# ascentai/diy-gym

Measured on NVIDIA B200. Metric: aggregate env-steps/sec, higher is better.
Workload: dtype f32

## Files before the change

### diy_gym_b200/csrc/dg_env.cuh

```cuda
#pragma once
#include "dg_math.cuh"
#include "dg_scene.h"

namespace dg {

struct Env {
  const DevScene* sc;
  float* ws;
  float* wg;
  float* st;
  float* pr;
  const float* act;
  float* obs;
  float* rew;
  uint8_t* term;
  const int* link_i;
  const float* link_f;
  const float* link_x;
  uint32_t seed;
  int env_id;
  bool active;
  int grp0, grp1;
  unsigned long long opmask[2];
  unsigned long long* dbg;
// ... 58 lines not shown
    float* K = KIN(s);
    q_to_mat(K, ST(S_BQUAT) + 4 * f); v_cpy(K + 9, ST(S_BPOS) + 3 * f);
  }
  if (ln == 0) for (int i = 0; i < WH_COUNT; i++) WSI(C)[sc.W_HDR + i] = 0;
}

DG_FN void joint_xform(const Env& C, int gl, float q, float* E, float* r) {
  const int* li = shc(C.link_i) + DG_LINK_I_W * gl; const float* lf = shc(C.link_f) + DG_LINK_F_W * gl; const float* R0 = shc(C.link_x) + 16 * gl;
  float Rrel[9], tmp[3];
  if (li[2] == 1) { float Ra[9]; axis_angle_mat(Ra, lf + 10, q, C.sc->precise != 0); m_mul(Rrel, R0, Ra); m_vec(tmp, Rrel, lf + 7); }
  else if (li[2] == 2) { m_cpy(Rrel, R0); float dd[3] = {lf[7] + lf[10] * q, lf[8] + lf[11] * q, lf[9] + lf[12] * q}; m_vec(tmp, R0, dd); }
  else { m_cpy(Rrel, R0); m_vec(tmp, R0, lf + 7); }
  v_add(r, lf + 4, tmp);
  E[0] = Rrel[0]; E[1] = Rrel[3]; E[2] = Rrel[6]; E[3] = Rrel[1]; E[4] = Rrel[4]; E[5] = Rrel[7]; E[6] = Rrel[2]; E[7] = Rrel[5]; E[8] = Rrel[8];
}
DG_HD int parent_slot(const int* li, int l0, int s0) { return li[1] < 0 ? s0 : s0 + 1 + (li[1] - l0); }

struct F4 { float x, y, z, w; };
DG_HD F4 ld4(const float* p) {
#if defined(__CUDA_ARCH__)
  float4 v = *reinterpret_cast<const float4*>(p); F4 o = {v.x, v.y, v.z, v.w}; return o;
#else
  F4 o = {p[0], p[1], p[2], p[3]}; return o;
#endif
}
DG_HD void st4(float* p, float x, float y, float z, float w) {
#if defined(__CUDA_ARCH__)
  *reinterpret_cast<float4*>(p) = make_float4(x, y, z, w);
#else
  p[0] = x; p[1] = y; p[2] = z; p[3] = w;
#endif
}
template <int N> DG_HD void ldn(const float* p, float* o) {
#pragma unroll
  for (int c = 0; c < N / 4; c++) { F4 v = ld4(p + 4 * c); o[4 * c] = v.x; o[4 * c + 1] = v.y; o[4 * c + 2] = v.z; o[4 * c + 3] = v.w; }
}
template <int N> DG_HD void stn(float* p, const float* v) {
#pragma unroll
  for (int c = 0; c < N / 4; c++) st4(p + 4 * c, v[4 * c], v[4 * c + 1], v[4 * c + 2], v[4 * c + 3]);
}

template <bool BIAS>
DG_FN void fk_vel_body(const Env& C, int b) {
  const DevScene& sc = SC;
  const int* bi = gc(sc.body_i) + DG_BODY_I_W * b; const int* bp = gc(sc.body_plan) + BP_W * b;
  const int kind = bi[0], l0 = bi[1], nlb = bi[2], s0 = bp[BP_SLOT];
  const float* bs = BST(bp[BP_DI]);
  const float *mass = PR(P_MASS), *inertia = PR(P_INERTIA);
  const float kl = PR(P_LINDAMP)[b], ka = PR(P_ANGDAMP)[b];
  float Kp[12], Vp[6];
  q_to_mat(Kp, bs + 3); v_cpy(Kp + 9, bs);
  mT_vec(Vp, Kp, bs + 10); mT_vec(Vp + 3, Kp, bs + 7);
  int prev = s0;
  for (int k = -1; k < nlb; k++) {
    const int s = s0 + 1 + k, f = k < 0 ? b : sc.nb + l0 + k;
    float K[12], V[6], cacc[8] = {0, 0, 0, 0, 0, 0, 0, 0};
    if (k < 0) {
      for (int i = 0; i < 12; i++) K[i] = Kp[i];
      for (int i = 0; i < 6; i++) V[i] = Vp[i];
    } else {
      const int gl = l0 + k; const int* li = shc(C.link_i) + DG_LINK_I_W * gl; const float* lx = shc(C.link_x) + 16 * gl;
      const int ps = parent_slot(li, l0, s0), dof = li[3];
      if (ps != prev) { ldn<12>(KIN(ps), Kp); const float* pv = ABA(ps) + AB_WV; for (int i = 0; i < 6; i++) Vp[i] = pv[i]; }
      float E[9], r[3], t[3], t2[3];
      joint_xform(C, gl, dof >= 0 ? DOF(D_Q, dof) : 0.f, E, r);
      float* L = LNK(gl);
      st4(L, E[0], E[1], E[2], E[3]); st4(L + 4, E[4], E[5], E[6], E[7]); st4(L + 8, E[8], r[0], r[1], r[2]);
      m_mulT(K, Kp, E);
      m_vec(t, Kp, r); v_add(K + 9, Kp + 9, t);
      m_vec(V, E, Vp);
      v_cross(t, Vp, r); v_add(t2, Vp + 3, t); m_vec(V + 3, E, t2);
      if (dof >= 0) {
        const float qd = DOF(D_QD, dof);
        if (BIAS) { float sa[3], sl[3]; v_scale(sa, lx + 9, qd); v_scale(sl, lx + 12, qd); v_cross(cacc, V, sa); v_cross(cacc + 3, V, sl); v_cross(t2, V + 3, sa); v_add(cacc + 3, cacc + 3, t2); }
        v_madd(V, lx + 9, qd); v_madd(V + 3, lx + 12, qd);
      }
      if (BIAS) stn<8>(LNX(gl), cacc);
    }
    stn<12>(KIN(s), K);
    float* X = ABA(s);
    if (!BIAS) {
      for (int i = 0; i < 6; i++) X[AB_WV + i] = V[i];
    } else if (k < 0 && kind != 2) {
      float z[40]; for (int i = 0; i < 40; i++) z[i] = 0.f;
      for (int i = 0; i < 6; i++) z[AB_WV + i] = V[i];
      stn<40>(X, z);
    } else {
      const float wsc = ((sc.sem & SEM_WRENCH_FIRST_SUBSTEP) && WSI(C)[sc.W_HDR + WH_SUB] > 0) ? 0.f : 1.f;
      const float efv[3] = {wsc * ST(S_EXTF)[3 * f], wsc * ST(S_EXTF)[3 * f + 1], wsc * ST(S_EXTF)[3 * f + 2]}, etv[3] = {wsc * ST(S_EXTT)[3 * f], wsc * ST(S_EXTT)[3 * f + 1], wsc * ST(S_EXTT)[3 * f + 2]};
      const float *ef = efv, *et = etv;
      const float m = mass[f]; const float* I = inertia + 3 * f; const float *w = V, *v = V + 3;
      float Iw[3] = {I[0] * w[0], I[1] * w[1], I[2] * w[2]}, t[3], fw[3], pa[3], pl[3];
      v_cross(pa, w, Iw);
      v_cross(t, w, v); v_scale(pl, t, m);
      fw[0] = sc.g[0] * m + ef[0]; fw[1] = sc.g[1] * m + ef[1]; fw[2] = sc.g[2] * m + ef[2];
      mT_vec(t, K, fw); v_sub(pl, pl, t);
      mT_vec(t, K, et); v_sub(pa, pa, t);
      const float wn = v_len(w), vn = v_len(v);
      const bool dlin = (sc.sem & SEM_DAMPING_LINEAR) != 0;
      v_madd(pa, Iw, dlin ? ka : ka + ka * wn);
      float mv[3]; v_scale(mv, v, m); v_madd(pl, mv, dlin ? kl : kl + kl * vn);
      float z[40]; for (int i = 0; i < 40; i++) z[i] = 0.f;
      for (int i = 0; i < 3; i++) { z[AB_PA + i] = pa[i]; z[AB_PA + 3 + i] = pl[i]; z[AB_WV + i] = w[i]; z[AB_WV + 3 + i] = v[i]; }
      z[AB_A] = I[0]; z[AB_A + 4] = I[1]; z[AB_A + 8] = I[2]; z[AB_C] = m; z[AB_C + 4] = m; z[AB_C + 8] = m;
      stn<40>(X, z);
    }
    for (int i = 0; i < 12; i++) Kp[i] = K[i];
    for (int i = 0; i < 6; i++) Vp[i] = V[i];
    prev = s;
  }
}

DG_HD void ia_mul(const float* A, const float* B, const float* Cm, const float* a, const float* l, float* n, float* f) {
  float t[3]; m_vec(n, A, a); m_vec(t, B, l); v_add(n, n, t); mT_vec(f, B, a); m_vec(t, Cm, l); v_add(f, f, t);
}
DG_FN int invert_small(float* M, int n, float* inv) {
  for (int i = 0; i < n; i++) for (int j = 0; j < n; j++) inv[i * n + j] = (i == j) ? 1.f : 0.f;
  for (int c = 0; c < n; c++) {
    int p = c;
    for (int r2 = c + 1; r2 < n; r2++) if (fabsf(M[r2 * n + c]) > fabsf(M[p * n + c])) p = r2;
    if (fabsf(M[p * n + c]) < 1e-30f) return -1;
// ... 37 lines not shown
    }
  }
#pragma unroll
  for (int i = 0; i < N; i++)
#pragma unroll
    for (int j = 0; j < N; j++) {
      float v = 0.f;
#pragma unroll
      for (int k = 0; k < N; k++) if (k >= i && k >= j) v += Li[k][i] * Li[k][j];
      Out[i][j] = v;
    }
}
DG_FN void aba_body(const Env& C, int b, float h) {
  const DevScene& sc = SC;
  const int* bi = gc(sc.body_i) + DG_BODY_I_W * b; const int* bp = gc(sc.body_plan) + BP_W * b;
  const int kind = bi[0], l0 = bi[1], nlb = bi[2], s0 = bp[BP_SLOT], di = bp[BP_DI];
  for (int k = nlb - 1; k >= 0; k--) {
    const int gl = l0 + k, s = s0 + 1 + k; const int* li = shc(C.link_i) + DG_LINK_I_W * gl;
    const int ps = parent_slot(li, l0, s0);
    float Xr[40], Lr[12], cx[8];
    ldn<40>(ABA(s), Xr); ldn<12>(LNK(gl), Lr); ldn<8>(LNX(gl), cx);
    float* Aa = Xr + AB_A; float* Ba = Xr + AB_B; float* Ca = Xr + AB_C; const float* pA = Xr + AB_PA;
    float pa[6], n[3], fo[3];
    if (li[3] >= 0) {
      const float* lx = shc(C.link_x) + 16 * gl; const float *sa = lx + 9, *sl = lx + 12;
      float U[6];
      ia_mul(Aa, Ba, Ca, sa, sl, U, U + 3);
      const float D = v_dot(sa, U) + v_dot(sl, U + 3);
      const float uu = DOF(D_TAU, li[3]) - (v_dot(sa, pA) + v_dot(sl, pA + 3));
      float* L = LNK(gl);
      st4(L + 12, U[0], U[1], U[2], U[3]); st4(L + 16, U[4], U[5], D, 0.f);
      LNX(gl)[6] = uu;
      const float Dinv = 1.0f / D;
#pragma unroll
// ... 44 lines not shown
    float iv[36];
#pragma unroll
    for (int i = 0; i < 6; i++)
#pragma unroll
      for (int j = 0; j < 6; j++) iv[6 * i + j] = Inv[i][j];
    stn<36>(Iv, iv);
#pragma unroll
    for (int i = 0; i < 6; i++) { float sum = 0.f;
#pragma unroll
      for (int j = 0; j < 6; j++) sum -= Inv[i][j] * Xr[AB_PA + j];
      a0[i] = sum; }
  } else for (int i = 0; i < 6; i++) a0[i] = 0.f;
#endif
  float ap[8]; int prev = s0;
  ldn<8>(a0, ap);
  for (int k = 0; k < nlb; k++) {
    const int gl = l0 + k, s = s0 + 1 + k; const int* li = shc(C.link_i) + DG_LINK_I_W * gl;
    const int ps = parent_slot(li, l0, s0);
    if (ps != prev) ldn<8>(ABA(ps) + AB_ACC, ap);
    float Lr[20], cx[8];
    ldn<20>(LNK(gl), Lr); ldn<8>(LNX(gl), cx);
    float t[3], t2[3], acc[8];
    m_vec(acc, Lr, ap); v_cross(t, ap, Lr + 9); v_add(t2, ap + 3, t); m_vec(acc + 3, Lr, t2);
    v_add(acc, acc, cx); v_add(acc + 3, acc + 3, cx + 3);
    if (li[3] >= 0) {
      const float* lx = shc(C.link_x) + 16 * gl;
      const float qdd = (cx[6] - (v_dot(Lr + 12, acc) + v_dot(Lr + 15, acc + 3))) / Lr[18];
      DOF(D_QD, li[3]) += h * qdd;
      v_madd(acc, lx + 9, qdd); v_madd(acc + 3, lx + 12, qdd);
    }
    acc[6] = 0.f; acc[7] = 0.f;
    stn<8>(ABA(s) + AB_ACC, acc);
    for (int i = 0; i < 8; i++) ap[i] = acc[i];
// ... 13 lines not shown
  for (int k = 0; k < nlb; k++) {
    float X[48], n[3], f[3];
    ldn<48>(ABA(s0 + 1 + k), X);
    ia_mul(X + AB_A, X + AB_B, X + AB_C, X + AB_ACC, X + AB_ACC + 3, n, f);
    float* o = ST(S_JREACT) + 6 * (l0 + k);
    for (int i = 0; i < 3; i++) { o[i] = X[AB_PA + 3 + i] + f[i]; o[3 + i] = X[AB_PA + i] + n[i]; }
  }
}
DG_FN void phase_dynamics(const Env& C, int ln, int nt, float h) {
  for (int di = ln; di < SC.ndyn; di += nt) { int b = gc(SC.dyn_body)[di]; fk_vel_body<true>(C, b); aba_body(C, b, h); if (SC.need_react) joint_reactions(C, b); }
}

DG_FN void minv_column(const Env& C, int b, int col, float* scr) {
  const DevScene& sc = SC;
  const int* bi = gc(sc.body_i) + DG_BODY_I_W * b; const int* bp = gc(sc.body_plan) + BP_W * b;
  const int kind = bi[0], l0 = bi[1], nlb = bi[2], d0 = bi[3], s0 = bp[BP_SLOT], g = bp[BP_GDIM], gs = bp[BP_GS];
  const int jo = kind == 2 ? 6 : 0;
  float* out = WSH(C, sc.W_MINV) + bp[BP_MINVOFF] + col * gs;
  for (int i = g; i < gs; i++) out[i] = 0.f;
  (void)scr;
  float uu[DG_MINV_MAXL], ast[6 * DG_MINV_MAXD];
  for (int k = 0; k < nlb; k++) uu[k] = 0.f;
  float p[6] = {0, 0, 0, 0, 0, 0};
  if (col >= jo) {
    int k0 = -1;
    for (int k = 0; k < nlb; k++) if (shc(C.link_i)[DG_LINK_I_W * (l0 + k) + 3] == d0 + col - jo) { k0 = k; break; }
    for (int k = k0; k >= 0;) {
      const int gl = l0 + k; const int* li = shc(C.link_i) + DG_LINK_I_W * gl;
      float L[20]; ldn<20>(LNK(gl), L);
      float pa[6] = {p[0], p[1], p[2], p[3], p[4], p[5]};
      if (li[3] >= 0) {
        const float* lx = shc(C.link_x) + 16 * gl;
        const float u1 = (k == k0 ? 1.f : 0.f) - (v_dot(lx + 9, pa) + v_dot(lx + 12, pa + 3));
        uu[k] = u1; const float s = u1 / L[18];
        for (int i = 0; i < 6; i++) pa[i] += L[12 + i] * s;
      }
      float fp[3], np_[3], t[3];
      mT_vec(fp, L, pa + 3); mT_vec(np_, L, pa); v_cross(t, L + 9, fp); v_add(np_, np_, t);
      v_cpy(p, np_); v_cpy(p + 3, fp);
      k = li[1] < 0 ? -1 : li[1] - l0;
    }
  }
  float a0[6];
  if (kind == 2) {
    float K0[12]; ldn<12>(KIN(s0), K0); const float* Iv = WSG(C, sc.W_I0) + bp[BP_I0OFF];
    float gen[6] = {0, 0, 0, 0, 0, 0}, rhs[6], t[3];
    for (int i = 0; i < 6; i++) gen[i] = (i == col) ? 1.f : 0.f;
    mT_vec(t, K0, gen); v_sub(rhs, t, p); mT_vec(t, K0, gen + 3); v_sub(rhs + 3, t, p + 3);
    for (int i = 0; i < 6; i++) { float s = 0.f; for (int j = 0; j < 6; j++) s += Iv[6 * i + j] * rhs[j]; a0[i] = s; }
    m_vec(out, K0, a0); m_vec(out + 3, K0, a0 + 3);
  } else for (int i = 0; i < 6; i++) a0[i] = 0.f;
  for (int i = 0; i < 6; i++) ast[i] = a0[i];
  float ap[6] = {a0[0], a0[1], a0[2], a0[3], a0[4], a0[5]}; int prev_dep = -1;
  for (int k = 0; k < nlb; k++) {
    const int gl = l0 + k; const int* li = shc(C.link_i) + DG_LINK_I_W * gl;
    const int dep = gc(sc.link_depth)[gl];
    if (dep - 1 != prev_dep) { const float* src = ast + 6 * dep; for (int i = 0; i < 6; i++) ap[i] = src[i]; }
    float L[20]; ldn<20>(LNK(gl), L);
    float t[3], t2[3], aa[3], al[3];
    m_vec(aa, L, ap); v_cross(t, ap, L + 9); v_add(t2, ap + 3, t); m_vec(al, L, t2);
    if (li[3] >= 0) {
      const float* lx = shc(C.link_x) + 16 * gl;
      const float qdd = (uu[k] - (v_dot(L + 12, aa) + v_dot(L + 15, al))) / L[18];
      out[jo + li[3] - d0] = qdd;
      v_madd(aa, lx + 9, qdd); v_madd(al, lx + 12, qdd);
    }
    float* ak = ast + 6 * (dep + 1);
    v_cpy(ak, aa); v_cpy(ak + 3, al);
    v_cpy(ap, aa); v_cpy(ap + 3, al); prev_dep = dep;
  }
}
// ... 329 lines not shown
DG_FN void point_jacobian(const Env& C, int f, const float* p, const float* dir, float* J) {
  const DevScene& sc = SC;
  int b = body_of_frame(C, f); const int* bi = gc(sc.body_i) + DG_BODY_I_W * b; const int* bp = gc(sc.body_plan) + BP_W * b;
  int g = bp[BP_GDIM], d0 = bi[3], s0 = bp[BP_SLOT], l0 = bi[1];
  for (int i = 0; i < g; i++) J[i] = 0.f;
  int jo = 0;
  if (bi[0] == 2) { float rel[3]; v_sub(rel, p, KIN(s0) + 9); v_cross(J, rel, dir); v_cpy(J + 3, dir); jo = 6; }
  int gl = f < sc.nb ? -1 : f - sc.nb;
  while (gl >= 0) {
    const int* li = shc(C.link_i) + DG_LINK_I_W * gl; const float* lf = shc(C.link_f) + DG_LINK_F_W * gl; const float* K = KIN(s0 + 1 + gl - l0);
    if (li[2] == 1) {
      float aw[3], dw[3], o[3], rel[3], t[3];
      m_vec(aw, K, lf + 10); m_vec(dw, K, lf + 7); v_sub(o, K + 9, dw);
      v_sub(rel, p, o); v_cross(t, aw, rel); J[jo + li[3] - d0] = v_dot(dir, t);
    } else if (li[2] == 2) { float aw[3]; m_vec(aw, K, lf + 10); J[jo + li[3] - d0] = v_dot(dir, aw); }
    gl = li[1];
  }
}
DG_FN void angular_jacobian(const Env& C, int f, const float* dir, float* J) {
  const DevScene& sc = SC;
  int b = body_of_frame(C, f); const int* bi = gc(sc.body_i) + DG_BODY_I_W * b; const int* bp = gc(sc.body_plan) + BP_W * b;
  int g = bp[BP_GDIM], d0 = bi[3], s0 = bp[BP_SLOT], l0 = bi[1], jo = 0;
  for (int i = 0; i < g; i++) J[i] = 0.f;
  if (bi[0] == 2) { v_cpy(J, dir); jo = 6; }
  for (int gl = f < sc.nb ? -1 : f - sc.nb; gl >= 0; gl = shc(C.link_i)[DG_LINK_I_W * gl + 1]) {
    const int* li = shc(C.link_i) + DG_LINK_I_W * gl;
    if (li[2] == 1) { float aw[3]; m_vec(aw, KIN(s0 + 1 + gl - l0), shc(C.link_f) + DG_LINK_F_W * gl + 10); J[jo + li[3] - d0] = v_dot(dir, aw); }
  }
}
DG_FN void body_genvel(const Env& C, int b, float* gv) {
  const int* bi = gc(SC.body_i) + DG_BODY_I_W * b; int jo = 0;
  if (bi[0] == 2) { const float* bs = BST(gc(SC.body_plan)[BP_W * b + BP_DI]); v_cpy(gv, bs + 10); v_cpy(gv + 3, bs + 7); jo = 6; }
  for (int i = 0; i < bi[4]; i++) gv[jo + i] = DOF(D_QD, bi[3] + i);
}
DG_FN void phase_unit_rows(const Env& C, int ln, int nt, float h) {
  const DevScene& sc = SC;
  for (int di = ln; di < sc.ndyn; di += nt) {
    int b = gc(sc.dyn_body)[di]; const int* bi = gc(sc.body_i) + DG_BODY_I_W * b; const int* bp = gc(sc.body_plan) + BP_W * b;
    int l0 = bi[1], nlb = bi[2], d0 = bi[3], g = bp[BP_GDIM], gs = bp[BP_GS], jo = bi[0] == 2 ? 6 : 0;
    const float* Minv = WSH(C, sc.W_MINV) + bp[BP_MINVOFF];
// ... 1172 lines not shown
```

### diy_gym_b200/csrc/dg_scene.h

```cpp
#pragma once
#include <stdint.h>

#include "scene_sections.h"

namespace dg {

enum { D_Q = 0, D_QD, D_APPLIED, D_TAU, D_COUNT };
enum { BP_DI = 0, BP_GDIM, BP_GVOFF, BP_MINVOFF, BP_I0OFF, BP_SLOT, BP_UROW, BP_DEPTH, BP_NRS, BP_AOFF, BP_GS, BP_W };
enum { WH_NCONTACT = 0, WH_NCROW, WH_NSURV, WH_COUPLED, WH_RS_R, WH_RS_NU, WH_RS_K, WH_RS_NEED, WH_RS_DEFER, WH_SUB, WH_COUNT = 12 };
enum { ST_ACT = 1, ST_PRE = 2, ST_POST = 4, ST_END = 8, ST_LOADC = 16, ST_SAVEC = 32, ST_LOAD = 128, ST_ALL = 15 };
enum { RS_NCLS = 3 };
enum { DG_MINV_MAXL = 64, DG_MINV_MAXD = 24 };
enum { RS_CONTACT = 0x40000000, RS_KMAX = 8, RS_GVMAX = 128 };
enum { RR_RHS = 0, RR_DINV, RR_LO, RR_HI, RR_MU, RR_PAR, RR_APPLIED, RR_ID, RR_W = 8 };
enum { UR_RHS = 0, UR_DINV, UR_LO, UR_HI, UR_APPLIED, UR_COL, UR_MOTOR, UR_W = 8 };
enum { CR_RHS = 0, CR_DINV, CR_LO, CR_HI, CR_APPLIED, CR_MU, CR_DA, CR_DB, CR_PARENT, CR_HDR = 12 };
enum { LK_W = 20, AB_PA = 0, AB_WV = 6, AB_A = 12, AB_B = 21, AB_C = 30, AB_ACC = 40, AB_W = 48, LX_W = 8 };
enum { CT_FA = 0, CT_FB, CT_PA = 2, CT_PB = 5, CT_N = 8, CT_DIST = 11, CT_MU = 12, CT_W = 13 };

struct DevScene {
  int nb, nl, nd, ns, nv, npair, ncam, nop, nframes, S, P, substeps, iters, maxc, hot_start, ik_iters;
  int n_act, n_obs, n_rew, n_term;
  int so[24];
  int po[12];
  float dt, g[3], erp, cerp, slop, margin, ik_damping, ik_threshold, max_joint_vel, limit_max_impulse, ik_null_lambda_sq;
  const int *body_i, *link_i, *shape_i, *pair_i, *vis_i, *op_i, *oparg_i, *cam_i;
  const float *body_f, *link_f, *shape_f, *vis_f, *oparg_f, *cam_f, *param_def, *state_def;
  const float* hull_f;
  int ndyn, nslot, nshw, nfloat, GD, GP, max_depth, max_nlb, n_ik, team;
  const int* dyn_body;
  const int* body_plan;
  const int* frame_slot;
  const int* link_depth;
  const int* shape_slot;
  const float* shape_wb;
  const float* vis_wb;
  const float* link_x;
  int ngrp, nloose;
  const int* grp_i;
  const int* grp_pairs;
  const int* loose_pairs;
  const float* body_reach;
  int w_total, g_total, ws_mode;
  int W_HDR, W_BST, W_DOF, W_EXT, W_KIN, W_LINK, W_MINV, W_DV, W_I0, W_UCNT, W_CAPP, W_X;
  int X_ABA, X_LNK, X_I0T;
  int X_SHW, X_CON, X_SURV, X_CTMP, X_UROW, X_CROW, X_MSCR, X_AMAT, X_IK, X_RSA, X_RSAS, X_RSV, X_RSREC;
  int GV;
  int rs_ashared;
  int rs_cap;
  int ncons;
  const int* cons_i; const float* cons_f;
  int need_react;
// ... 1 lines not shown
  int rs_cls_k[RS_NCLS], rs_cls_r[RS_NCLS];
  int solver;
  int crow_stride, mscr_stride, ctmp_stride, ik_stride;
  int sem;
  int precise;
};

#define DG_SO(sc, name) ((sc)->so[HI_##name - HI_S_BPOS])
#define DG_PO(sc, name) ((sc)->po[HI_##name - HI_P_MASS])

}

#ifndef __CUDACC_RTC__
#include <algorithm>
#include <cmath>
#include <string>
#include <vector>

namespace dg {

struct HostScene {
  std::vector<int> ints;
  std::vector<float> floats;
  DevScene dev;
  std::string error;

  struct Off { size_t body_i, link_i, shape_i, pair_i, vis_i, op_i, oparg_i, cam_i, dyn_body, body_plan, frame_slot, link_depth, shape_slot, grp_i, grp_pairs, loose_pairs;
               size_t body_f, link_f, shape_f, vis_f, oparg_f, cam_f, param_def, state_def, shape_wb, vis_wb, link_x, body_reach, cons_i, cons_f, hull_f; } off;

  static void quat_to_mat(const double* q, double* m) {
    double x = q[0], y = q[1], z = q[2], w = q[3];
    double n = 1.0 / std::sqrt(x * x + y * y + z * z + w * w); x *= n; y *= n; z *= n; w *= n;
    m[0] = 1 - 2 * (y * y + z * z); m[1] = 2 * (x * y - z * w); m[2] = 2 * (x * z + y * w);
    m[3] = 2 * (x * y + z * w); m[4] = 1 - 2 * (x * x + z * z); m[5] = 2 * (y * z - x * w);
    m[6] = 2 * (x * z - y * w); m[7] = 2 * (y * z + x * w); m[8] = 1 - 2 * (x * x + y * y);
  }

  void point(DevScene& d, const int* ib, const float* fb) const {
    d.body_i = ib + off.body_i; d.link_i = ib + off.link_i; d.shape_i = ib + off.shape_i; d.pair_i = ib + off.pair_i;
    d.vis_i = ib + off.vis_i; d.op_i = ib + off.op_i; d.oparg_i = ib + off.oparg_i; d.cam_i = ib + off.cam_i;
    d.dyn_body = ib + off.dyn_body; d.body_plan = ib + off.body_plan; d.frame_slot = ib + off.frame_slot;
    d.link_depth = ib + off.link_depth; d.shape_slot = ib + off.shape_slot;
    d.grp_i = ib + off.grp_i; d.grp_pairs = ib + off.grp_pairs; d.loose_pairs = ib + off.loose_pairs; d.body_reach = fb + off.body_reach;
    d.body_f = fb + off.body_f; d.link_f = fb + off.link_f; d.shape_f = fb + off.shape_f; d.vis_f = fb + off.vis_f;
    d.oparg_f = fb + off.oparg_f; d.cam_f = fb + off.cam_f; d.param_def = fb + off.param_def; d.state_def = fb + off.state_def;
    d.shape_wb = fb + off.shape_wb; d.vis_wb = fb + off.vis_wb; d.link_x = fb + off.link_x;
    d.cons_i = ib + off.cons_i; d.cons_f = fb + off.cons_f; d.hull_f = fb + off.hull_f;
  }

  bool build(const int32_t* ibuf, int ni, const double* fbuf, int nf, int team, int ws_mode = 0, int rs_ashared = 0) {
    if (ni < 2 + 3 * DG_NSECTIONS || ibuf[0] != (int32_t)DG_SCENE_MAGIC || ibuf[1] != DG_NSECTIONS) { error = "bad scene magic / section count"; return false; }
    auto sec_off = [&](int s) { return (size_t)ibuf[2 + 3 * s + 1]; };
    auto sec_len = [&](int s) { return (size_t)ibuf[2 + 3 * s + 2]; };
    for (int s = 0; s < DG_NSECTIONS; s++) {
      bool is_f = ibuf[2 + 3 * s] != 0;
      if (sec_off(s) + sec_len(s) > (size_t)(is_f ? nf : ni)) { error = "section out of range"; return false; }
    }
    const int32_t* hi = ibuf + sec_off(SEC_HDR_I);
    const double* hf = fbuf + sec_off(SEC_HDR_F);
    DevScene& d = dev;
    d = DevScene();
    d.nb = hi[HI_nb]; d.nl = hi[HI_nl]; d.nd = hi[HI_nd]; d.ns = hi[HI_ns]; d.nv = hi[HI_nv]; d.npair = hi[HI_npair];
    d.ncam = hi[HI_ncam]; d.nop = hi[HI_nop]; d.nframes = hi[HI_nframes]; d.S = hi[HI_S]; d.P = hi[HI_P];
    d.substeps = hi[HI_substeps]; d.iters = hi[HI_iterations]; d.maxc = hi[HI_max_contacts]; d.hot_start = hi[HI_hot_start];
    d.ik_iters = hi[HI_ik_iters]; d.n_act = hi[HI_n_act]; d.n_obs = hi[HI_n_obs]; d.n_rew = hi[HI_n_rew]; d.n_term = hi[HI_n_term];
// ... 69 lines not shown
    std::vector<float> link_x((size_t)std::max(d.nl, 1) * 16, 0.f);
    {
      const double* link_f = fbuf + sec_off(SEC_LINK_F);
      for (int gl = 0; gl < d.nl; gl++) {
        const double* lf = link_f + DG_LINK_F_W * gl; int jt = link_i[DG_LINK_I_W * gl + 2];
        double m[9]; quat_to_mat(lf, m);
        for (int i = 0; i < 9; i++) link_x[16 * gl + i] = (float)m[i];
        const double *a = lf + 10, *dd = lf + 7;
        if (jt == 1) {
          for (int i = 0; i < 3; i++) link_x[16 * gl + 9 + i] = (float)a[i];
          link_x[16 * gl + 12] = (float)(a[1] * dd[2] - a[2] * dd[1]); link_x[16 * gl + 13] = (float)(a[2] * dd[0] - a[0] * dd[2]);
          link_x[16 * gl + 14] = (float)(a[0] * dd[1] - a[1] * dd[0]);
        } else if (jt == 2) for (int i = 0; i < 3; i++) link_x[16 * gl + 12 + i] = (float)a[i];
      }
    }
    std::vector<float> body_reach(d.nb, 0.f);
    {
      const double* link_f = fbuf + sec_off(SEC_LINK_F);
      std::vector<double> lreach(std::max(d.nl, 1), 0.0);
      auto norm3 = [](const double* v) { return std::sqrt(v[0] * v[0] + v[1] * v[1] + v[2] * v[2]); };
      for (int gl = 0; gl < d.nl; gl++) {
        const double* lf = link_f + DG_LINK_F_W * gl; const int32_t* li = link_i + DG_LINK_I_W * gl;
        double travel = li[2] == 2 ? std::max(std::fabs(lf[20]), std::fabs(lf[21])) : 0.0;
        lreach[gl] = (li[1] < 0 ? 0.0 : lreach[li[1]]) + norm3(lf + 4) + norm3(lf + 7) + travel;
      }
      for (int s = 0; s < d.ns; s++) {
        int b = shape_i[DG_SHAPE_I_W * s], f = shape_i[DG_SHAPE_I_W * s + 1];
        double r = (f < d.nb ? 0.0 : lreach[f - d.nb]) + norm3(shape_f + DG_SHAPE_F_W * s) + shape_f[DG_SHAPE_F_W * s + 11];
        body_reach[b] = std::max(body_reach[b], (float)(r * 1.0001 + 1e-6));
      }
// ... 11 lines not shown
        long long key = (long long)stat * d.nb + dynb; size_t g = 0;
        for (; g < keys.size(); g++) if (keys[g] == key) break;
        if (g == keys.size()) { keys.push_back(key); members.emplace_back(); }
        members[g].push_back(k);
      }
      for (size_t g = 0; g < keys.size(); g++) {
        grp_i.push_back((int)(keys[g] / d.nb)); grp_i.push_back((int)(keys[g] % d.nb)); grp_i.push_back((int)grp_pairs.size()); grp_i.push_back((int)members[g].size());
        grp_pairs.insert(grp_pairs.end(), members[g].begin(), members[g].end());
      }
    }
    int GP = 1;
    auto gdim_of_shape = [&](int s) { int b = shape_i[DG_SHAPE_I_W * s]; return body_plan[(size_t)b * BP_W + BP_GDIM]; };
    for (int k = 0; k < d.npair; k++) GP = std::max(GP, gdim_of_shape(pair_i[2 * k]) + gdim_of_shape(pair_i[2 * k + 1]));
    int n_ik = 0;
    for (int k = 0; k < d.nop; k++) n_ik += op_i[DG_OP_I_W * k] == OP_IK_CTRL;
    d.need_react = hi[HI_S_STEP] > hi[HI_S_JREACT];
    d.precise = d.ncons > 0; d.sem = hi[HI_semantics];

    auto put_vi = [&](const std::vector<int>& v) { size_t o = ints.size(); ints.insert(ints.end(), v.begin(), v.end()); ints.push_back(0); return o; };
    auto put_vf = [&](const std::vector<float>& v) { size_t o = floats.size(); floats.insert(floats.end(), v.begin(), v.end()); floats.push_back(0.f); return o; };
    off.dyn_body = put_vi(dyn_body); off.body_plan = put_vi(body_plan); off.frame_slot = put_vi(frame_slot);
    off.link_depth = put_vi(link_depth); off.shape_slot = put_vi(shape_slot);
    off.shape_wb = put_vf(shape_wb); off.vis_wb = put_vf(vis_wb); off.link_x = put_vf(link_x); off.body_reach = put_vf(body_reach);
    off.grp_i = put_vi(grp_i); off.grp_pairs = put_vi(grp_pairs); off.loose_pairs = put_vi(loose_pairs);
    point(d, ints.data(), floats.data());

    d.ndyn = (int)dyn_body.size(); d.nslot = nslot; d.nshw = nshw; d.nfloat = nfloat; d.GD = GD; d.GP = GP;
    if (max_nlb > DG_MINV_MAXL || max_depth + 2 > DG_MINV_MAXD) { error = "a body has more than " + std::to_string((int)DG_MINV_MAXL) + " links or a kinematic tree deeper than " + std::to_string((int)DG_MINV_MAXD - 2); return false; }
    d.max_depth = max_depth; d.max_nlb = max_nlb; d.n_ik = n_ik; d.ngrp = (int)grp_i.size() / 4; d.nloose = (int)loose_pairs.size();

    enum { RC_SMALL = 0, RC_KIN, RC_ABA, RC_SOLVE, RC_CONTACT, RC_SCRATCH };
    auto is_cold = [&](int rc) {
      if (rc == RC_SMALL || rc == RC_SOLVE) return false;
      if (rc == RC_KIN || rc == RC_ABA || rc == RC_SCRATCH) return true;
      return ws_mode == 3;
    };
    int fix[2] = {0, 0};
    int ph[2][3] = {{0, 0, 0}, {0, 0, 0}};
    auto enc_rc = [&](int rc, int cold, int off) { return (rc == RC_CONTACT && cold) ? ~off : off; };
    auto take = [&](int rc, int n) { int c = is_cold(rc); int r = fix[c]; fix[c] += (n + 3) & ~3; return std::make_pair(c, r); };
    auto fixed = [&](int rc, int n) { auto pr = take(rc, n); return enc_rc(rc, pr.first, pr.second); };
    d.W_HDR = fixed(RC_SMALL, WH_COUNT);
    d.W_BST = fixed(RC_SMALL, 13 * d.ndyn);
// ... 57 lines not shown
```

Baseline: 2.563 million.

## Fold fixed links into movable parents for articulated-body recursion

Precomputes on the host a folded kinematic tree in which fixed (zero-DOF) links are merged into their nearest movable ancestor, with composed transforms and an inertia lumped onto that ancestor. FK, ABA passes, the mass-matrix inverse columns and the Jacobians then iterate only over movable links, while folded frames still get their kinematics and velocities written for downstream use. The aim is to cut per-link recursion work and memory traffic for robots with many fixed links. The fold is on by default, can be turned off with DG_FOLD, and is skipped when joint reactions are needed; it adds a parallel-axis inertia accumulation and per-frame bias transforms.

```diff
diff --git a/diy_gym_b200/csrc/dg_env.cuh b/diy_gym_b200/csrc/dg_env.cuh
--- a/diy_gym_b200/csrc/dg_env.cuh
+++ b/diy_gym_b200/csrc/dg_env.cuh
@@ -96,7 +96,17 @@
   v_add(r, lf + 4, tmp);
   E[0] = Rrel[0]; E[1] = Rrel[3]; E[2] = Rrel[6]; E[3] = Rrel[1]; E[4] = Rrel[4]; E[5] = Rrel[7]; E[6] = Rrel[2]; E[7] = Rrel[5]; E[8] = Rrel[8];
 }
-DG_HD int parent_slot(const int* li, int l0, int s0) { return li[1] < 0 ? s0 : s0 + 1 + (li[1] - l0); }
+DG_FN void joint_xform_folded(const Env& C, int gl, float q, float* E, float* r) {
+  const int* li = shc(C.link_i) + DG_LINK_I_W * gl; const float* lf = shc(C.link_f) + DG_LINK_F_W * gl; const float* R0 = gc(C.sc->fold_x) + 12 * gl;
+  float Rrel[9], tmp[3];
+  if (li[2] == 1) { float Ra[9]; axis_angle_mat(Ra, lf + 10, q, C.sc->precise != 0); m_mul(Rrel, R0, Ra); m_vec(tmp, Rrel, lf + 7); }
+  else if (li[2] == 2) { m_cpy(Rrel, R0); float dd[3] = {lf[7] + lf[10] * q, lf[8] + lf[11] * q, lf[9] + lf[12] * q}; m_vec(tmp, R0, dd); }
+  else { m_cpy(Rrel, R0); m_vec(tmp, R0, lf + 7); }
+  v_add(r, R0 + 9, tmp);
+  E[0] = Rrel[0]; E[1] = Rrel[3]; E[2] = Rrel[6]; E[3] = Rrel[1]; E[4] = Rrel[4]; E[5] = Rrel[7]; E[6] = Rrel[2]; E[7] = Rrel[5]; E[8] = Rrel[8];
+}
+DG_HD int fold_up(const DevScene& sc, int gl) { return gc(sc.fold_i)[FI_W * gl + FI_UP]; }
+DG_HD int fold_parent_slot(const DevScene& sc, int gl, int l0, int s0) { const int u = fold_up(sc, gl); return u < 0 ? s0 : s0 + 1 + (u - l0); }
 
 struct F4 { float x, y, z, w; };
 DG_HD F4 ld4(const float* p) {
@@ -122,30 +132,49 @@
   for (int c = 0; c < N / 4; c++) st4(p + 4 * c, v[4 * c], v[4 * c + 1], v[4 * c + 2], v[4 * c + 3]);
 }
 
+DG_FN void frame_bias(const Env& C, int f, const float* K, const float* V, float wsc, float kl, float ka, float* pa, float* pl) {
+  const DevScene& sc = SC;
+  const float efv[3] = {wsc * ST(S_EXTF)[3 * f], wsc * ST(S_EXTF)[3 * f + 1], wsc * ST(S_EXTF)[3 * f + 2]}, etv[3] = {wsc * ST(S_EXTT)[3 * f], wsc * ST(S_EXTT)[3 * f + 1], wsc * ST(S_EXTT)[3 * f + 2]};
+  const float *ef = efv, *et = etv;
+  const float m = PR(P_MASS)[f]; const float* I = PR(P_INERTIA) + 3 * f; const float *w = V, *v = V + 3;
+  float Iw[3] = {I[0] * w[0], I[1] * w[1], I[2] * w[2]}, t[3], fw[3];
+  v_cross(pa, w, Iw);
+  v_cross(t, w, v); v_scale(pl, t, m);
+  fw[0] = sc.g[0] * m + ef[0]; fw[1] = sc.g[1] * m + ef[1]; fw[2] = sc.g[2] * m + ef[2];
+  mT_vec(t, K, fw); v_sub(pl, pl, t);
+  mT_vec(t, K, et); v_sub(pa, pa, t);
+  const float wn = v_len(w), vn = v_len(v);
+  const bool dlin = (sc.sem & SEM_DAMPING_LINEAR) != 0;
+  v_madd(pa, Iw, dlin ? ka : ka + ka * wn);
+  float mv[3]; v_scale(mv, v, m); v_madd(pl, mv, dlin ? kl : kl + kl * vn);
+}
+
 template <bool BIAS>
-DG_FN void fk_vel_body(const Env& C, int b) {
+DG_NOINLINE DG_FN void fk_vel_body(const Env& C, int b) {
   const DevScene& sc = SC;
   const int* bi = gc(sc.body_i) + DG_BODY_I_W * b; const int* bp = gc(sc.body_plan) + BP_W * b;
-  const int kind = bi[0], l0 = bi[1], nlb = bi[2], s0 = bp[BP_SLOT];
+  const int kind = bi[0], l0 = bi[1], s0 = bp[BP_SLOT], m0 = bp[BP_MOV0], nmov = bp[BP_NMOV];
   const float* bs = BST(bp[BP_DI]);
   const float *mass = PR(P_MASS), *inertia = PR(P_INERTIA);
   const float kl = PR(P_LINDAMP)[b], ka = PR(P_ANGDAMP)[b];
+  const float wsc = ((sc.sem & SEM_WRENCH_FIRST_SUBSTEP) && WSI(C)[sc.W_HDR + WH_SUB] > 0) ? 0.f : 1.f;
   float Kp[12], Vp[6];
   q_to_mat(Kp, bs + 3); v_cpy(Kp + 9, bs);
   mT_vec(Vp, Kp, bs + 10); mT_vec(Vp + 3, Kp, bs + 7);
   int prev = s0;
-  for (int k = -1; k < nlb; k++) {
-    const int s = s0 + 1 + k, f = k < 0 ? b : sc.nb + l0 + k;
+  for (int k = -1; k < nmov; k++) {
+    const int gl = k < 0 ? -1 : gc(sc.fold_list)[m0 + k];
+    const int s = k < 0 ? s0 : s0 + 1 + (gl - l0), f = k < 0 ? b : sc.nb + gl;
     float K[12], V[6], cacc[8] = {0, 0, 0, 0, 0, 0, 0, 0};
     if (k < 0) {
       for (int i = 0; i < 12; i++) K[i] = Kp[i];
       for (int i = 0; i < 6; i++) V[i] = Vp[i];
     } else {
-      const int gl = l0 + k; const int* li = shc(C.link_i) + DG_LINK_I_W * gl; const float* lx = shc(C.link_x) + 16 * gl;
-      const int ps = parent_slot(li, l0, s0), dof = li[3];
+      const int* li = shc(C.link_i) + DG_LINK_I_W * gl; const float* lx = shc(C.link_x) + 16 * gl;
+      const int ps = fold_parent_slot(sc, gl, l0, s0), dof = li[3];
       if (ps != prev) { ldn<12>(KIN(ps), Kp); const float* pv = ABA(ps) + AB_WV; for (int i = 0; i < 6; i++) Vp[i] = pv[i]; }
       float E[9], r[3], t[3], t2[3];
-      joint_xform(C, gl, dof >= 0 ? DOF(D_Q, dof) : 0.f, E, r);
+      joint_xform_folded(C, gl, dof >= 0 ? DOF(D_Q, dof) : 0.f, E, r);
       float* L = LNK(gl);
       st4(L, E[0], E[1], E[2], E[3]); st4(L + 4, E[4], E[5], E[6], E[7]); st4(L + 8, E[8], r[0], r[1], r[2]);
       m_mulT(K, Kp, E);
@@ -161,32 +190,44 @@
     }
     stn<12>(KIN(s), K);
     float* X = ABA(s);
-    if (!BIAS) {
-      for (int i = 0; i < 6; i++) X[AB_WV + i] = V[i];
-    } else if (k < 0 && kind != 2) {
-      float z[40]; for (int i = 0; i < 40; i++) z[i] = 0.f;
+    const bool rec = BIAS && (k >= 0 || kind == 2);
+    float z[40];
+    if (BIAS) {
+      for (int i = 0; i < 40; i++) z[i] = 0.f;
       for (int i = 0; i < 6; i++) z[AB_WV + i] = V[i];
-      stn<40>(X, z);
-    } else {
-      const float wsc = ((sc.sem & SEM_WRENCH_FIRST_SUBSTEP) && WSI(C)[sc.W_HDR + WH_SUB] > 0) ? 0.f : 1.f;
-      const float efv[3] = {wsc * ST(S_EXTF)[3 * f], wsc * ST(S_EXTF)[3 * f + 1], wsc * ST(S_EXTF)[3 * f + 2]}, etv[3] = {wsc * ST(S_EXTT)[3 * f], wsc * ST(S_EXTT)[3 * f + 1], wsc * ST(S_EXTT)[3 * f + 2]};
-      const float *ef = efv, *et = etv;
-      const float m = mass[f]; const float* I = inertia + 3 * f; const float *w = V, *v = V + 3;
-      float Iw[3] = {I[0] * w[0], I[1] * w[1], I[2] * w[2]}, t[3], fw[3], pa[3], pl[3];
-      v_cross(pa, w, Iw);
-      v_cross(t, w, v); v_scale(pl, t, m);
-      fw[0] = sc.g[0] * m + ef[0]; fw[1] = sc.g[1] * m + ef[1]; fw[2] = sc.g[2] * m + ef[2];
-      mT_vec(t, K, fw); v_sub(pl, pl, t);
-      mT_vec(t, K, et); v_sub(pa, pa, t);
-      const float wn = v_len(w), vn = v_len(v);
-      const bool dlin = (sc.sem & SEM_DAMPING_LINEAR) != 0;
-      v_madd(pa, Iw, dlin ? ka : ka + ka * wn);
-      float mv[3]; v_scale(mv, v, m); v_madd(pl, mv, dlin ? kl : kl + kl * vn);
-      float z[40]; for (int i = 0; i < 40; i++) z[i] = 0.f;
-      for (int i = 0; i < 3; i++) { z[AB_PA + i] = pa[i]; z[AB_PA + 3 + i] = pl[i]; z[AB_WV + i] = w[i]; z[AB_WV + 3 + i] = v[i]; }
+    }
+    if (rec) {
+      const float m = mass[f]; const float* I = inertia + 3 * f;
+      frame_bias(C, f, K, V, wsc, kl, ka, z + AB_PA, z + AB_PA + 3);
       z[AB_A] = I[0]; z[AB_A + 4] = I[1]; z[AB_A + 8] = I[2]; z[AB_C] = m; z[AB_C + 4] = m; z[AB_C + 8] = m;
-      stn<40>(X, z);
-    }
+    }
+    const int* fl = k < 0 ? bp + BP_FL0 : gc(sc.fold_i) + FI_W * gl + FI_FL0;
+    for (int j = 0; j < fl[1]; j++) {
+      const int gf = gc(sc.fold_list)[fl[0] + j], sf = s0 + 1 + (gf - l0);
+      const float* fx = gc(sc.fold_x) + 12 * gf; const float* ph = fx + 9;
+      float Kf[12], Vf[6], t[3], t2[3];
+      m_mul(Kf, K, fx); m_vec(t, K, ph); v_add(Kf + 9, K + 9, t);
+      mT_vec(Vf, fx, V); v_cross(t, V, ph); v_add(t2, V + 3, t); mT_vec(Vf + 3, fx, t2);
+      stn<12>(KIN(sf), Kf);
+      float* Xf = ABA(sf) + AB_WV;
+      for (int i = 0; i < 6; i++) Xf[i] = Vf[i];
+      if (rec) {
+        float pa[3], pl[3], fp[3], np_[3];
+        frame_bias(C, sc.nb + gf, Kf, Vf, wsc, kl, ka, pa, pl);
+        m_vec(fp, fx, pl); m_vec(np_, fx, pa); v_cross(t, ph, fp); v_add(np_, np_, t);
+        for (int i = 0; i < 3; i++) { z[AB_PA + i] += np_[i]; z[AB_PA + 3 + i] += fp[i]; }
+        const float m = mass[sc.nb + gf]; const float* I = inertia + 3 * (sc.nb + gf); const float pp = v_dot(ph, ph);
+#pragma unroll
+        for (int r = 0; r < 3; r++)
+#pragma unroll
+          for (int c = 0; c < 3; c++)
+            z[AB_A + 3 * r + c] += fx[3 * r] * I[0] * fx[3 * c] + fx[3 * r + 1] * I[1] * fx[3 * c + 1] + fx[3 * r + 2] * I[2] * fx[3 * c + 2] + m * ((r == c ? pp : 0.f) - ph[r] * ph[c]);
+        z[AB_B + 1] -= m * ph[2]; z[AB_B + 2] += m * ph[1]; z[AB_B + 3] += m * ph[2]; z[AB_B + 5] -= m * ph[0]; z[AB_B + 6] -= m * ph[1]; z[AB_B + 7] += m * ph[0];
+        z[AB_C] += m; z[AB_C + 4] += m; z[AB_C + 8] += m;
+      }
+    }
+    if (BIAS) stn<40>(X, z);
+    else for (int i = 0; i < 6; i++) X[AB_WV + i] = V[i];
     for (int i = 0; i < 12; i++) Kp[i] = K[i];
     for (int i = 0; i < 6; i++) Vp[i] = V[i];
     prev = s;
@@ -254,10 +295,10 @@
 DG_FN void aba_body(const Env& C, int b, float h) {
   const DevScene& sc = SC;
   const int* bi = gc(sc.body_i) + DG_BODY_I_W * b; const int* bp = gc(sc.body_plan) + BP_W * b;
-  const int kind = bi[0], l0 = bi[1], nlb = bi[2], s0 = bp[BP_SLOT], di = bp[BP_DI];
-  for (int k = nlb - 1; k >= 0; k--) {
-    const int gl = l0 + k, s = s0 + 1 + k; const int* li = shc(C.link_i) + DG_LINK_I_W * gl;
-    const int ps = parent_slot(li, l0, s0);
+  const int kind = bi[0], l0 = bi[1], s0 = bp[BP_SLOT], di = bp[BP_DI], m0 = bp[BP_MOV0], nmov = bp[BP_NMOV];
+  for (int k = nmov - 1; k >= 0; k--) {
+    const int gl = gc(sc.fold_list)[m0 + k], s = s0 + 1 + (gl - l0); const int* li = shc(C.link_i) + DG_LINK_I_W * gl;
+    const int ps = fold_parent_slot(sc, gl, l0, s0);
     float Xr[40], Lr[12], cx[8];
     ldn<40>(ABA(s), Xr); ldn<12>(LNK(gl), Lr); ldn<8>(LNX(gl), cx);
     float* Aa = Xr + AB_A; float* Ba = Xr + AB_B; float* Ca = Xr + AB_C; const float* pA = Xr + AB_PA;
@@ -332,9 +373,9 @@
 #endif
   float ap[8]; int prev = s0;
   ldn<8>(a0, ap);
-  for (int k = 0; k < nlb; k++) {
-    const int gl = l0 + k, s = s0 + 1 + k; const int* li = shc(C.link_i) + DG_LINK_I_W * gl;
-    const int ps = parent_slot(li, l0, s0);
+  for (int k = 0; k < nmov; k++) {
+    const int gl = gc(sc.fold_list)[m0 + k], s = s0 + 1 + (gl - l0); const int* li = shc(C.link_i) + DG_LINK_I_W * gl;
+    const int ps = fold_parent_slot(sc, gl, l0, s0);
     if (ps != prev) ldn<8>(ABA(ps) + AB_ACC, ap);
     float Lr[20], cx[8];
     ldn<20>(LNK(gl), Lr); ldn<8>(LNX(gl), cx);
@@ -378,17 +419,17 @@
 DG_FN void minv_column(const Env& C, int b, int col, float* scr) {
   const DevScene& sc = SC;
   const int* bi = gc(sc.body_i) + DG_BODY_I_W * b; const int* bp = gc(sc.body_plan) + BP_W * b;
-  const int kind = bi[0], l0 = bi[1], nlb = bi[2], d0 = bi[3], s0 = bp[BP_SLOT], g = bp[BP_GDIM], gs = bp[BP_GS];
+  const int kind = bi[0], l0 = bi[1], d0 = bi[3], s0 = bp[BP_SLOT], g = bp[BP_GDIM], gs = bp[BP_GS], m0 = bp[BP_MOV0], nmov = bp[BP_NMOV];
   const int jo = kind == 2 ? 6 : 0;
   float* out = WSH(C, sc.W_MINV) + bp[BP_MINVOFF] + col * gs;
   for (int i = g; i < gs; i++) out[i] = 0.f;
   (void)scr;
   float uu[DG_MINV_MAXL], ast[6 * DG_MINV_MAXD];
-  for (int k = 0; k < nlb; k++) uu[k] = 0.f;
+  for (int k = 0; k < nmov; k++) uu[gc(sc.fold_list)[m0 + k] - l0] = 0.f;
   float p[6] = {0, 0, 0, 0, 0, 0};
   if (col >= jo) {
     int k0 = -1;
-    for (int k = 0; k < nlb; k++) if (shc(C.link_i)[DG_LINK_I_W * (l0 + k) + 3] == d0 + col - jo) { k0 = k; break; }
+    for (int k = 0; k < nmov; k++) { const int gl = gc(sc.fold_list)[m0 + k]; if (shc(C.link_i)[DG_LINK_I_W * gl + 3] == d0 + col - jo) { k0 = gl - l0; break; } }
     for (int k = k0; k >= 0;) {
       const int gl = l0 + k; const int* li = shc(C.link_i) + DG_LINK_I_W * gl;
       float L[20]; ldn<20>(LNK(gl), L);
@@ -402,7 +443,8 @@
       float fp[3], np_[3], t[3];
       mT_vec(fp, L, pa + 3); mT_vec(np_, L, pa); v_cross(t, L + 9, fp); v_add(np_, np_, t);
       v_cpy(p, np_); v_cpy(p + 3, fp);
-      k = li[1] < 0 ? -1 : li[1] - l0;
+      const int up = fold_up(sc, gl);
+      k = up < 0 ? -1 : up - l0;
     }
   }
   float a0[6];
@@ -416,9 +458,9 @@
   } else for (int i = 0; i < 6; i++) a0[i] = 0.f;
   for (int i = 0; i < 6; i++) ast[i] = a0[i];
   float ap[6] = {a0[0], a0[1], a0[2], a0[3], a0[4], a0[5]}; int prev_dep = -1;
-  for (int k = 0; k < nlb; k++) {
-    const int gl = l0 + k; const int* li = shc(C.link_i) + DG_LINK_I_W * gl;
-    const int dep = gc(sc.link_depth)[gl];
+  for (int m = 0; m < nmov; m++) {
+    const int gl = gc(sc.fold_list)[m0 + m], k = gl - l0; const int* li = shc(C.link_i) + DG_LINK_I_W * gl;
+    const int dep = gc(sc.fold_i)[FI_W * gl + FI_DEP];
     if (dep - 1 != prev_dep) { const float* src = ast + 6 * dep; for (int i = 0; i < 6; i++) ap[i] = src[i]; }
     float L[20]; ldn<20>(LNK(gl), L);
     float t[3], t2[3], aa[3], al[3];
@@ -778,7 +820,7 @@
       m_vec(aw, K, lf + 10); m_vec(dw, K, lf + 7); v_sub(o, K + 9, dw);
       v_sub(rel, p, o); v_cross(t, aw, rel); J[jo + li[3] - d0] = v_dot(dir, t);
     } else if (li[2] == 2) { float aw[3]; m_vec(aw, K, lf + 10); J[jo + li[3] - d0] = v_dot(dir, aw); }
-    gl = li[1];
+    gl = fold_up(sc, gl);
   }
 }
 DG_FN void angular_jacobian(const Env& C, int f, const float* dir, float* J) {
@@ -787,7 +829,7 @@
   int g = bp[BP_GDIM], d0 = bi[3], s0 = bp[BP_SLOT], l0 = bi[1], jo = 0;
   for (int i = 0; i < g; i++) J[i] = 0.f;
   if (bi[0] == 2) { v_cpy(J, dir); jo = 6; }
-  for (int gl = f < sc.nb ? -1 : f - sc.nb; gl >= 0; gl = shc(C.link_i)[DG_LINK_I_W * gl + 1]) {
+  for (int gl = f < sc.nb ? -1 : f - sc.nb; gl >= 0; gl = fold_up(sc, gl)) {
     const int* li = shc(C.link_i) + DG_LINK_I_W * gl;
     if (li[2] == 1) { float aw[3]; m_vec(aw, KIN(s0 + 1 + gl - l0), shc(C.link_f) + DG_LINK_F_W * gl + 10); J[jo + li[3] - d0] = v_dot(dir, aw); }
   }
diff --git a/diy_gym_b200/csrc/dg_scene.h b/diy_gym_b200/csrc/dg_scene.h
--- a/diy_gym_b200/csrc/dg_scene.h
+++ b/diy_gym_b200/csrc/dg_scene.h
@@ -6,7 +6,8 @@
 namespace dg {
 
 enum { D_Q = 0, D_QD, D_APPLIED, D_TAU, D_COUNT };
-enum { BP_DI = 0, BP_GDIM, BP_GVOFF, BP_MINVOFF, BP_I0OFF, BP_SLOT, BP_UROW, BP_DEPTH, BP_NRS, BP_AOFF, BP_GS, BP_W };
+enum { BP_DI = 0, BP_GDIM, BP_GVOFF, BP_MINVOFF, BP_I0OFF, BP_SLOT, BP_UROW, BP_DEPTH, BP_NRS, BP_AOFF, BP_GS, BP_MOV0, BP_NMOV, BP_FL0, BP_NFL, BP_FDEPTH, BP_W };
+enum { FI_UP = 0, FI_FL0, FI_NFL, FI_DEP, FI_W = 4 };
 enum { WH_NCONTACT = 0, WH_NCROW, WH_NSURV, WH_COUPLED, WH_RS_R, WH_RS_NU, WH_RS_K, WH_RS_NEED, WH_RS_DEFER, WH_SUB, WH_COUNT = 12 };
 enum { ST_ACT = 1, ST_PRE = 2, ST_POST = 4, ST_END = 8, ST_LOADC = 16, ST_SAVEC = 32, ST_LOAD = 128, ST_ALL = 15 };
 enum { RS_NCLS = 3 };
@@ -36,6 +37,10 @@
   const float* shape_wb;
   const float* vis_wb;
   const float* link_x;
+  int fold;
+  const int* fold_i;
+  const int* fold_list;
+  const float* fold_x;
   int ngrp, nloose;
   const int* grp_i;
   const int* grp_pairs;
@@ -67,6 +72,7 @@
 #ifndef __CUDACC_RTC__
 #include <algorithm>
 #include <cmath>
+#include <cstdlib>
 #include <string>
 #include <vector>
 
@@ -78,8 +84,8 @@
   DevScene dev;
   std::string error;
 
-  struct Off { size_t body_i, link_i, shape_i, pair_i, vis_i, op_i, oparg_i, cam_i, dyn_body, body_plan, frame_slot, link_depth, shape_slot, grp_i, grp_pairs, loose_pairs;
-               size_t body_f, link_f, shape_f, vis_f, oparg_f, cam_f, param_def, state_def, shape_wb, vis_wb, link_x, body_reach, cons_i, cons_f, hull_f; } off;
+  struct Off { size_t body_i, link_i, shape_i, pair_i, vis_i, op_i, oparg_i, cam_i, dyn_body, body_plan, frame_slot, link_depth, shape_slot, grp_i, grp_pairs, loose_pairs, fold_i, fold_list;
+               size_t body_f, link_f, shape_f, vis_f, oparg_f, cam_f, param_def, state_def, shape_wb, vis_wb, link_x, body_reach, cons_i, cons_f, hull_f, fold_x; } off;
 
   static void quat_to_mat(const double* q, double* m) {
     double x = q[0], y = q[1], z = q[2], w = q[3];
@@ -99,9 +105,11 @@
     d.oparg_f = fb + off.oparg_f; d.cam_f = fb + off.cam_f; d.param_def = fb + off.param_def; d.state_def = fb + off.state_def;
     d.shape_wb = fb + off.shape_wb; d.vis_wb = fb + off.vis_wb; d.link_x = fb + off.link_x;
     d.cons_i = ib + off.cons_i; d.cons_f = fb + off.cons_f; d.hull_f = fb + off.hull_f;
+    d.fold_i = ib + off.fold_i; d.fold_list = ib + off.fold_list; d.fold_x = fb + off.fold_x;
   }
 
-  bool build(const int32_t* ibuf, int ni, const double* fbuf, int nf, int team, int ws_mode = 0, int rs_ashared = 0) {
+  bool build(const int32_t* ibuf, int ni, const double* fbuf, int nf, int team, int ws_mode = 0, int rs_ashared = 0, int fold = -1) {
+    if (fold < 0) { const char* ef = std::getenv("DG_FOLD"); fold = ef ? std::atoi(ef) != 0 : 1; }
     if (ni < 2 + 3 * DG_NSECTIONS || ibuf[0] != (int32_t)DG_SCENE_MAGIC || ibuf[1] != DG_NSECTIONS) { error = "bad scene magic / section count"; return false; }
     auto sec_off = [&](int s) { return (size_t)ibuf[2 + 3 * s + 1]; };
     auto sec_len = [&](int s) { return (size_t)ibuf[2 + 3 * s + 2]; };
@@ -201,6 +209,68 @@
         } else if (jt == 2) for (int i = 0; i < 3; i++) link_x[16 * gl + 12 + i] = (float)a[i];
       }
     }
+    d.need_react = hi[HI_S_STEP] > hi[HI_S_JREACT];
+    d.fold = fold && !d.need_react;
+    std::vector<int> fold_i((size_t)std::max(d.nl, 1) * FI_W, 0), fold_list;
+    std::vector<float> fold_x((size_t)std::max(d.nl, 1) * 12, 0.f);
+    int max_fdepth = 0;
+    {
+      const double* link_f = fbuf + sec_off(SEC_LINK_F);
+      std::vector<double> hx((size_t)std::max(d.nl, 1) * 12, 0.0);
+      std::vector<int> folded(std::max(d.nl, 1), 0);
+      auto mul33 = [](double* o, const double* a, const double* b) {
+        for (int i = 0; i < 3; i++) for (int j = 0; j < 3; j++) o[3 * i + j] = a[3 * i] * b[j] + a[3 * i + 1] * b[3 + j] + a[3 * i + 2] * b[6 + j];
+      };
+      auto affine = [](double* o, const double* R, const double* p, const double* v) {
+        for (int i = 0; i < 3; i++) o[i] = p[i] + R[3 * i] * v[0] + R[3 * i + 1] * v[1] + R[3 * i + 2] * v[2];
+      };
+      for (int b = 0; b < d.nb; b++) {
+        const int32_t* bi = body_i + DG_BODY_I_W * b; int* bp = &body_plan[(size_t)b * BP_W];
+        const int kind = bi[0], l0 = bi[1], nlb = bi[2], fold_b = d.fold && kind != 0 && bi[4] > 0;
+        bp[BP_MOV0] = (int)fold_list.size();
+        for (int k = 0; k < nlb; k++) {
+          const int gl = l0 + k, pl = link_i[DG_LINK_I_W * gl + 1], dof = link_i[DG_LINK_I_W * gl + 3];
+          const double* lf = link_f + DG_LINK_F_W * gl;
+          double Rp[9] = {1, 0, 0, 0, 1, 0, 0, 0, 1}, pp[3] = {0, 0, 0};
+          int* fi = &fold_i[(size_t)FI_W * gl];
+          fi[FI_UP] = pl;
+          if (pl >= 0 && folded[pl]) {
+            for (int i = 0; i < 9; i++) Rp[i] = hx[12 * pl + i];
+            for (int i = 0; i < 3; i++) pp[i] = hx[12 * pl + 9 + i];
+            fi[FI_UP] = fold_i[(size_t)FI_W * pl + FI_UP];
+          }
+          double R0[9], RR[9]; quat_to_mat(lf, R0); mul33(RR, Rp, R0);
+          if (fold_b && dof < 0) {
+            double r[3]; affine(r, R0, lf + 4, lf + 7);
+            folded[gl] = 1;
+            for (int i = 0; i < 9; i++) hx[12 * gl + i] = RR[i];
+            affine(&hx[12 * gl + 9], Rp, pp, r);
+            for (int i = 0; i < 12; i++) fold_x[12 * gl + i] = (float)hx[12 * gl + i];
+          } else {
+            fold_list.push_back(gl);
+            fi[FI_DEP] = fi[FI_UP] < 0 ? 0 : fold_i[(size_t)FI_W * fi[FI_UP] + FI_DEP] + 1;
+            max_fdepth = std::max(max_fdepth, fi[FI_DEP]);
+            double o[3]; affine(o, Rp, pp, lf + 4);
+            for (int i = 0; i < 9; i++) fold_x[12 * gl + i] = (float)RR[i];
+            for (int i = 0; i < 3; i++) fold_x[12 * gl + 9 + i] = (float)o[i];
+          }
+        }
+        bp[BP_NMOV] = (int)fold_list.size() - bp[BP_MOV0];
+        int fdepth = 0;
+        for (int m = 0; m < bp[BP_NMOV]; m++) fdepth = std::max(fdepth, fold_i[(size_t)FI_W * fold_list[bp[BP_MOV0] + m] + FI_DEP]);
+        bp[BP_FDEPTH] = fdepth;
+        auto collect = [&](int host) {
+          int n = 0;
+          for (int k = 0; k < nlb; k++) if (folded[l0 + k] && fold_i[(size_t)FI_W * (l0 + k) + FI_UP] == host) { fold_list.push_back(l0 + k); n++; }
+          return n;
+        };
+        bp[BP_FL0] = (int)fold_list.size(); bp[BP_NFL] = collect(-1);
+        for (int m = 0; m < bp[BP_NMOV]; m++) {
+          const int gl = fold_list[bp[BP_MOV0] + m]; int* fi = &fold_i[(size_t)FI_W * gl];
+          fi[FI_FL0] = (int)fold_list.size(); fi[FI_NFL] = collect(gl);
+        }
+      }
+    }
     std::vector<float> body_reach(d.nb, 0.f);
     {
       const double* link_f = fbuf + sec_off(SEC_LINK_F);
@@ -242,7 +312,6 @@
     for (int k = 0; k < d.npair; k++) GP = std::max(GP, gdim_of_shape(pair_i[2 * k]) + gdim_of_shape(pair_i[2 * k + 1]));
     int n_ik = 0;
     for (int k = 0; k < d.nop; k++) n_ik += op_i[DG_OP_I_W * k] == OP_IK_CTRL;
-    d.need_react = hi[HI_S_STEP] > hi[HI_S_JREACT];
     d.precise = d.ncons > 0; d.sem = hi[HI_semantics];
 
     auto put_vi = [&](const std::vector<int>& v) { size_t o = ints.size(); ints.insert(ints.end(), v.begin(), v.end()); ints.push_back(0); return o; };
@@ -251,10 +320,11 @@
     off.link_depth = put_vi(link_depth); off.shape_slot = put_vi(shape_slot);
     off.shape_wb = put_vf(shape_wb); off.vis_wb = put_vf(vis_wb); off.link_x = put_vf(link_x); off.body_reach = put_vf(body_reach);
     off.grp_i = put_vi(grp_i); off.grp_pairs = put_vi(grp_pairs); off.loose_pairs = put_vi(loose_pairs);
+    off.fold_i = put_vi(fold_i); off.fold_list = put_vi(fold_list); off.fold_x = put_vf(fold_x);
     point(d, ints.data(), floats.data());
 
     d.ndyn = (int)dyn_body.size(); d.nslot = nslot; d.nshw = nshw; d.nfloat = nfloat; d.GD = GD; d.GP = GP;
-    if (max_nlb > DG_MINV_MAXL || max_depth + 2 > DG_MINV_MAXD) { error = "a body has more than " + std::to_string((int)DG_MINV_MAXL) + " links or a kinematic tree deeper than " + std::to_string((int)DG_MINV_MAXD - 2); return false; }
+    if (max_nlb > DG_MINV_MAXL || max_fdepth + 2 > DG_MINV_MAXD) { error = "a body has more than " + std::to_string((int)DG_MINV_MAXL) + " links or more than " + std::to_string((int)DG_MINV_MAXD - 2) + " movable links on one path from its base"; return false; }
     d.max_depth = max_depth; d.max_nlb = max_nlb; d.n_ik = n_ik; d.ngrp = (int)grp_i.size() / 4; d.nloose = (int)loose_pairs.size();
 
     enum { RC_SMALL = 0, RC_KIN, RC_ABA, RC_SOLVE, RC_CONTACT, RC_SCRATCH };
```

New measurement: 2.638 million, median of 6. 2.9% higher.
